# neka-nat/cupoch

Hardware: NVIDIA H100
Metric: icp_iterations_per_sec (higher is better)
Workload: dtype f32

## Files before the change

### cupoch_b200/csrc/icp.cu

```cuda
#include <float.h>
#include <math.h>
#include <stddef.h>
#include <stdlib.h>
#include <time.h>
#include <string.h>

#include "cphb_internal.cuh"
#include <vector>
#include "cphb_eigen3.cuh"

#include "icp_types.cuh"
#include "icp_solve.cuh"
#include "icp_rows.cuh"
#include "icp_kernels.cuh"
#include "icp_estimate.cuh"
#include "icp_aux.cuh"


struct cphb_icp {
    cphb_index *index;
    cphb_icp_params prm;
    cphb_cloud tgt;
    unsigned n_src, n_pad;
    unsigned n_full;
    void *arena;
    size_t arena_bytes;
    float4 *pristine_xyz, *pristine_nrm, *pristine_cov;
    float4 *work_xyz, *work_nrm, *work_cov;
    float4 *src_col;
    float4 *tix_nrm, *tix_grad, *tix_cov;
    float4 *alt_xyz, *alt_nrm, *alt_cov, *alt_col, *cur_col;
    int2 *alt_prev;
    uint32_t *rt_keys, *rt_keys2, *rt_vals, *rt_order;
    IcpState *st;
    IcpState *h_st;
    bool owns_host;
    cudaEvent_t ev0, ev1;
    double *partials;
    int32_t *corr_index;
    unsigned *cmp_counts;
    unsigned *cmp_total;
    double *tile_sums;
    unsigned *flag_bits;
    unsigned flag_words;
    int2 *prev;
    unsigned *dbg = nullptr;
    cudaEvent_t *dbg_ev = nullptr;
    unsigned grid_search;
    unsigned grid;
    unsigned reduce_grid;
    cudaStream_t stream;
};

struct HostCache {
    IcpState *h_st = nullptr;
    cudaEvent_t ev0 = nullptr, ev1 = nullptr;
    bool in_use = false;
};
static thread_local HostCache t_cache;
static thread_local cudaEvent_t t_source_ready = nullptr;
struct SideStream {
    cudaStream_t stream = nullptr;
    cudaEvent_t fork = nullptr, join = nullptr;
    int device = -1;
};
static thread_local SideStream t_side;

static bool is_identity4(const float *T) {
// ... 193 lines not shown
    }
    const bool want_nrm = params->estimation == CPHB_EST_SYMMETRIC && source->normals;
    const bool want_col = params->estimation == CPHB_EST_COLORED_ICP && source->colors;
    const bool want_cov = params->estimation == CPHB_EST_GENERALIZED_ICP && source->covariances;
    size_t off = 0;
    auto take = [&](size_t bytes) { size_t o = off; off = cphb_align(off + bytes, 256); return o; };
    size_t o_pxyz = take(sizeof(float4) * n_pad), o_wxyz = take(sizeof(float4) * n_pad);
    size_t o_pnrm = want_nrm ? take(sizeof(float4) * n_pad) : 0, o_wnrm = want_nrm ? take(sizeof(float4) * n_pad) : 0;
    size_t o_pcov = want_cov ? take(sizeof(float4) * 3 * n_pad) : 0, o_wcov = want_cov ? take(sizeof(float4) * 3 * n_pad) : 0;
    size_t o_col = want_col ? take(sizeof(float4) * n_pad) : 0;
    size_t o_st = take(sizeof(IcpState));
    size_t o_part = take(sizeof(double) * 32 * (icp->reduce_grid > icp->grid ? icp->reduce_grid : icp->grid));
    const size_t nt_pad = (size_t)icp->index->v.n_leaves * CPHB_LEAF;
    const int est = params->estimation;
    const bool t_nrm = target->normals && (est == CPHB_EST_POINT_TO_PLANE || est == CPHB_EST_SYMMETRIC || est == CPHB_EST_COLORED_ICP);
    const bool t_grad = target->color_gradient && est == CPHB_EST_COLORED_ICP;
    const bool t_cov = target->covariances && est == CPHB_EST_GENERALIZED_ICP;
    size_t o_tn = t_nrm ? take(sizeof(float4) * (nt_pad ? nt_pad : 1)) : 0, o_tg = t_grad ? take(sizeof(float4) * (nt_pad ? nt_pad : 1)) : 0;
    size_t o_tc = t_cov ? take(sizeof(float4) * 3 * (nt_pad ? nt_pad : 1)) : 0;
    size_t o_ts = take(sizeof(double) * n_pad);
    const unsigned flag_words = n_pad / 1024 + 1;
    size_t o_fb = take(sizeof(unsigned) * 2 * flag_words);
    size_t o_prev = take(sizeof(int2) * n_pad);
    size_t o_axyz = take(sizeof(float4) * n_pad), o_aprev = take(sizeof(int2) * n_pad);
    size_t o_anrm = want_nrm ? take(sizeof(float4) * n_pad) : 0, o_acov = want_cov ? take(sizeof(float4) * 3 * n_pad) : 0;
    size_t o_acol = want_col ? take(sizeof(float4) * n_pad) : 0, o_ccol = want_col ? take(sizeof(float4) * n_pad) : 0;
    size_t o_rt = take(sizeof(uint32_t) * 4 * n_pad);
    const unsigned nf_pad = (unsigned)cphb_align(n_full ? n_full : 1, ICP_BLOCK);
    size_t o_ci = take(sizeof(int32_t) * nf_pad);
    unsigned cmp_blocks = (nf_pad + CMP_BLOCK - 1) / CMP_BLOCK;
    size_t o_cc = take(sizeof(unsigned) * (cmp_blocks + 1));
    size_t o_ct = take(16);
    icp->arena_bytes = off;
    rc = cphb_alloc_async(&icp->arena, off, s);
    if (rc) { cphb_index_destroy(icp->index); delete icp; return rc; }
    char *b = (char *)icp->arena;
    icp->pristine_xyz = (float4 *)(b + o_pxyz);
    icp->work_xyz = (float4 *)(b + o_wxyz);
    icp->pristine_nrm = want_nrm ? (float4 *)(b + o_pnrm) : nullptr;
    icp->work_nrm = want_nrm ? (float4 *)(b + o_wnrm) : nullptr;
    icp->pristine_cov = want_cov ? (float4 *)(b + o_pcov) : nullptr;
    icp->work_cov = want_cov ? (float4 *)(b + o_wcov) : nullptr;
    icp->src_col = want_col ? (float4 *)(b + o_col) : nullptr;
    icp->st = (IcpState *)(b + o_st);
    icp->partials = (double *)(b + o_part);
    icp->tix_nrm = t_nrm ? (float4 *)(b + o_tn) : nullptr;
    icp->tix_grad = t_grad ? (float4 *)(b + o_tg) : nullptr;
    icp->tix_cov = t_cov ? (float4 *)(b + o_tc) : nullptr;
    icp->tile_sums = (double *)(b + o_ts);
    icp->flag_bits = (unsigned *)(b + o_fb);
    icp->flag_words = flag_words;
    icp->prev = (int2 *)(b + o_prev);
    icp->alt_xyz = (float4 *)(b + o_axyz);
    icp->alt_prev = (int2 *)(b + o_aprev);
    icp->alt_nrm = want_nrm ? (float4 *)(b + o_anrm) : nullptr;
    icp->alt_cov = want_cov ? (float4 *)(b + o_acov) : nullptr;
    icp->alt_col = want_col ? (float4 *)(b + o_acol) : nullptr;
    icp->cur_col = want_col ? (float4 *)(b + o_ccol) : nullptr;
    icp->rt_keys = (uint32_t *)(b + o_rt);
    icp->rt_keys2 = icp->rt_keys + n_pad;
    icp->rt_vals = icp->rt_keys + 2 * (size_t)n_pad;
    icp->rt_order = icp->rt_keys + 3 * (size_t)n_pad;
    icp->corr_index = (int32_t *)(b + o_ci);
    icp->cmp_counts = (unsigned *)(b + o_cc);
    icp->cmp_total = (unsigned *)(b + o_ct);
    if (!t_cache.in_use) {
        if (!t_cache.h_st) {
            CREATE_TRY(cudaMallocHost((void **)&t_cache.h_st, sizeof(IcpState)));
            CREATE_TRY(cudaEventCreate(&t_cache.ev0));
            CREATE_TRY(cudaEventCreate(&t_cache.ev1));
        }
        t_cache.in_use = true;
        icp->owns_host = false;
        icp->h_st = t_cache.h_st;
        icp->ev0 = t_cache.ev0;
// ... 39 lines not shown
    delete icp;
}

static void fill_args(const cphb_icp *icp, IcpArgs &a) {
    memset(&a, 0, sizeof(a));
    a.ix = icp->index->v;
    a.src = icp->work_xyz;
    a.src_nrm = icp->work_nrm;
    a.src_cov = icp->work_cov;
    a.src_col = icp->src_col;
    a.tgt_nrm = icp->tix_nrm;
    a.tgt_grad = icp->tix_grad;
    a.tgt_cov = icp->tix_cov;
    a.has_tgt_col = icp->tgt.colors != nullptr;
    a.st = icp->st;
    a.partials = icp->partials;
    a.tile_sums = icp->tile_sums;
    a.flag_bits = icp->flag_bits;
    a.flag_words = icp->flag_words;
    a.reduce_grid = icp->reduce_grid;
    a.helper_blocks = icp->grid >= 64 ? (icp->grid / 8 > 2 ? icp->grid / 8 : 2) : 0;
    if (const char *e = getenv("CPHB_HELPER_BLOCKS")) { int v = atoi(e); if (v >= 0 && (unsigned)v < icp->grid / 2) a.helper_blocks = (unsigned)v; }
    a.prev = icp->prev;
    a.n_src = icp->n_src;
    a.n_pad = icp->n_pad;
    a.n_total = icp->n_src;
    float r = icp->prm.max_correspondence_distance;
    a.r2 = (r > 0.f) ? r * r : 0.f;
    a.rel_fitness = icp->prm.relative_fitness;
    a.rel_rmse = icp->prm.relative_rmse;
    a.det_thresh = icp->prm.det_thresh;
    a.max_iter = icp->prm.max_iteration > 0 ? icp->prm.max_iteration : 0;
    float lg = icp->prm.lambda_geometric;
    if (lg < 0.f || lg > 1.0f) lg = 0.968f;
    a.sg = (float)sqrt((double)lg);
    float lp = (float)(1.0 - (double)lg);
    a.sp = (float)sqrt((double)lp);
    a.cert_gain = 4.f;
    a.cert_cap = 0.5f;
    if (const char *e = getenv("CPHB_CERT_GAIN")) a.cert_gain = (float)atof(e);
    if (const char *e = getenv("CPHB_CERT_CAP")) a.cert_cap = (float)atof(e);
    a.cert_cap_r = 0.25f * (r > 0.f ? r : 0.f);
    a.r_up = (float)(sqrt((double)a.r2) * 1.00002);
    a.dbg = icp->dbg;
    a.claim_max = 8u;
    if (const char *e = getenv("CPHB_CLAIM_MAX")) { int v = atoi(e); if (v >= 1 && v <= 1024) a.claim_max = (unsigned)v; }
// ... 22 lines not shown
    unsigned nb = (n + CMP_BLOCK - 1) / CMP_BLOCK;
    if (nb == 0) nb = 1;
    CPHB_LAUNCH(compact_count_kernel, nb, CMP_BLOCK, 0, s, icp->corr_index, n, icp->cmp_counts);
    CPHB_LAUNCH(compact_scan_kernel, 1, 1024, 0, s, icp->cmp_counts, nb, icp->cmp_total);
    CPHB_LAUNCH(compact_write_kernel, nb, CMP_BLOCK, 0, s, icp->corr_index, n, icp->cmp_counts, corr_out);
    CPHB_CHECK_LAUNCH();
    return CPHB_OK;
}

static int retile(cphb_icp *icp, IcpArgs &a, cudaStream_t s) {
    const unsigned n_pad = icp->n_pad, grid = n_pad / 256;
    const uint32_t n_tgt_pad = (uint32_t)icp->index->v.n_leaves * CPHB_LEAF;
    CPHB_LAUNCH(retile_key_kernel, grid, 256, 0, s, a.prev, icp->n_src, n_pad, n_tgt_pad, icp->rt_keys, icp->rt_vals);
    CPHB_CHECK_LAUNCH();
    int bits = 1;
    while (bits < 32 && ((uint64_t)1 << bits) < (uint64_t)(n_tgt_pad >> 5) + 2u) ++bits;
    int rc = cphb_sort_pairs_u32(icp->rt_keys, icp->rt_keys2, icp->rt_vals, icp->rt_order, n_pad, bits, s);
    if (rc) return rc;
    float4 *o_xyz = (a.src == icp->work_xyz) ? icp->alt_xyz : icp->work_xyz;
    int2 *o_prev = (a.prev == icp->prev) ? icp->alt_prev : icp->prev;
    float4 *o_nrm = a.src_nrm ? ((a.src_nrm == icp->work_nrm) ? icp->alt_nrm : icp->work_nrm) : nullptr;
    float4 *o_cov = a.src_cov ? ((a.src_cov == icp->work_cov) ? icp->alt_cov : icp->work_cov) : nullptr;
    float4 *o_col = a.src_col ? ((a.src_col == icp->alt_col) ? icp->cur_col : icp->alt_col) : nullptr;
    CPHB_LAUNCH(retile_gather_kernel, grid, 256, 0, s, icp->rt_order, n_pad, a.src, a.prev, a.src_nrm, a.src_col, a.src_cov,
                o_xyz, o_prev, o_nrm, o_col, o_cov);
    CPHB_CHECK_LAUNCH();
    a.src = o_xyz;
    a.prev = o_prev;
    a.src_nrm = o_nrm;
    a.src_cov = o_cov;
    a.src_col = o_col;
    return CPHB_OK;
}

extern "C" int cphb_icp_run(cphb_icp *icp, const float h_init[16], cphb_comm *comm, cphb_icp_result *h_result,
                            int32_t *corr_out, void *stream) {
    cudaStream_t s = (cudaStream_t)stream;
    if (!icp || !h_init || !h_result) {
        cphb_set_error("cphb_icp_run: null argument");
        return CPHB_ERR_INVALID;
    }
    int rc = reset_working_copy(icp, s);
    if (rc) return rc;
    IcpState *h = icp->h_st;
    memset(h, 0, sizeof(*h));
    memcpy(h->T, h_init, 64);
    memcpy(h->U, h_init, 64);
    h->apply_u = is_identity4(h_init) ? 0 : 1;
    CPHB_CUDA(cudaMemcpyAsync(icp->st, h, sizeof(IcpState), cudaMemcpyHostToDevice, s));
    static const bool dbg_cert = getenv("CPHB_DEBUG_CERT") != nullptr;
    if (dbg_cert) {
        if (!icp->dbg) CPHB_CUDA(cudaMalloc(&icp->dbg, sizeof(unsigned) * 256 + 128));
        CPHB_CUDA(cudaMemsetAsync(icp->dbg, 0, sizeof(unsigned) * 256 + 128, s));
        CPHB_CUDA(cudaMemsetAsync(icp->dbg + 256, 0xff, 8, s));
// ... 421 lines not shown
```

### cupoch_b200/csrc/icp_aux.cuh

```cuda
#pragma once

__global__ void __launch_bounds__(256) gather_source_kernel(const float *__restrict__ xyz, const float *__restrict__ nrm,
                                                            const float *__restrict__ col, const float *__restrict__ cov,
                                                            int cov_col_major, const uint32_t *__restrict__ perm_all,
                                                            unsigned lo, unsigned n, unsigned n_pad, float4 *o_xyz,
                                                            float4 *o_nrm, float4 *o_col, float4 *o_cov) {
    unsigned i = blockIdx.x * blockDim.x + threadIdx.x;
    if (i >= n_pad) return;
    const uint32_t *perm = perm_all + lo;
    if (i < n) {
        size_t j = perm[i];
        o_xyz[i] = make_float4(xyz[3 * j], xyz[3 * j + 1], xyz[3 * j + 2], __uint_as_float((unsigned)j));
        if (o_nrm) o_nrm[i] = make_float4(nrm[3 * j], nrm[3 * j + 1], nrm[3 * j + 2], 0.f);
        if (o_col) o_col[i] = make_float4(col[3 * j], col[3 * j + 1], col[3 * j + 2], 0.f);
        if (o_cov) {
            const float *c = cov + 9 * j;
            for (int r = 0; r < 3; ++r)
                o_cov[(size_t)r * n_pad + i] = cov_col_major ? make_float4(c[r], c[3 + r], c[6 + r], 0.f)
                                                             : make_float4(c[3 * r], c[3 * r + 1], c[3 * r + 2], 0.f);
        }
    } else {
        size_t j = n ? perm[n - 1] : 0;
        float4 p = n ? make_float4(xyz[3 * j], xyz[3 * j + 1], xyz[3 * j + 2], 0.f) : make_float4(0.f, 0.f, 0.f, 0.f);
        p.w = __uint_as_float(0xffffffffu);
// ... 28 lines not shown
#pragma unroll
        for (int r = 0; r < 3; ++r)
            o_cov[3 * p + r] = !real ? make_float4(0.f, 0.f, 0.f, 0.f)
                                     : cov_col_major ? make_float4(c[r], c[3 + r], c[6 + r], 0.f)
                                                     : make_float4(c[3 * r], c[3 * r + 1], c[3 * r + 2], 0.f);
    }
}

__global__ void __launch_bounds__(256) retile_key_kernel(const int2 *__restrict__ prev, unsigned n_src, unsigned n_pad,
                                                         uint32_t n_tgt_pad, uint32_t *keys, uint32_t *vals) {
    unsigned i = blockIdx.x * blockDim.x + threadIdx.x;
    if (i >= n_pad) return;
    uint32_t k = (n_tgt_pad >> 5) + 1u;
    if (i < n_src) {
        const int pp = prev[i].x;
        k = (pp >= 0) ? ((uint32_t)pp >> 5) : (n_tgt_pad >> 5);
    }
    keys[i] = k;
    vals[i] = i;
}
__global__ void __launch_bounds__(256) retile_gather_kernel(const uint32_t *__restrict__ order, unsigned n_pad,
                                                            const float4 *__restrict__ xyz, const int2 *__restrict__ prev,
                                                            const float4 *__restrict__ nrm, const float4 *__restrict__ col,
                                                            const float4 *__restrict__ cov, float4 *o_xyz, int2 *o_prev,
                                                            float4 *o_nrm, float4 *o_col, float4 *o_cov) {
    unsigned i = blockIdx.x * blockDim.x + threadIdx.x;
    if (i >= n_pad) return;
    const unsigned s = order[i];
    o_xyz[i] = xyz[s];
    o_prev[i] = prev[s];
    if (nrm) o_nrm[i] = nrm[s];
    if (col) o_col[i] = col[s];
    if (cov)
#pragma unroll
        for (int r = 0; r < 3; ++r) o_cov[(size_t)r * n_pad + i] = cov[(size_t)r * n_pad + s];
}

#define CMP_BLOCK 1024
__global__ void __launch_bounds__(CMP_BLOCK) compact_count_kernel(const int32_t *__restrict__ ci, unsigned n,
                                                                  unsigned *block_counts) {
    __shared__ unsigned s_w[32];
    unsigned i = blockIdx.x * CMP_BLOCK + threadIdx.x;
    bool v = i < n && ci[i] >= 0;
    unsigned m = __ballot_sync(CPHB_FULL, v);
    if (lane_id() == 0) s_w[threadIdx.x >> 5] = __popc(m);
    __syncthreads();
    if (threadIdx.x < 32) {
        unsigned c = s_w[threadIdx.x];
#pragma unroll
        for (int o = 16; o > 0; o >>= 1) c += __shfl_xor_sync(CPHB_FULL, c, o);
        if (threadIdx.x == 0) block_counts[blockIdx.x] = c;
    }
}
// ... 98 lines not shown
```

### cupoch_b200/csrc/icp_kernels.cuh

```cuda
#pragma once

__device__ __forceinline__ void prefetch_l1(const void *p) { asm volatile("prefetch.global.L1 [%0];" ::"l"(p)); }
__device__ __forceinline__ void cp_async_16(void *smem, const void *gmem) {
    asm volatile("cp.async.cg.shared.global [%0], [%1], 16;" ::"r"(smem_u32(smem)), "l"(gmem) : "memory");
}
__device__ __forceinline__ void cp_async_8(void *smem, const void *gmem) {
    asm volatile("cp.async.ca.shared.global [%0], [%1], 8;" ::"r"(smem_u32(smem)), "l"(gmem) : "memory");
}
__device__ __forceinline__ void cp_async_commit() { asm volatile("cp.async.commit_group;" ::: "memory"); }
__device__ __forceinline__ void cp_async_wait_0() { asm volatile("cp.async.wait_group 0;" ::: "memory"); }
template <int N>
__device__ __forceinline__ void cp_async_wait() { asm volatile("cp.async.wait_group %0;" ::"n"(N) : "memory"); }
#ifndef ICP_GD
#define ICP_GD 2
#endif
#define ICP_NS (2 * ICP_GD)
#ifndef ICP_DMMA
#define ICP_DMMA 1
#endif
#ifndef ICP_F2D_INT
#define ICP_F2D_INT 0
#endif
__device__ __forceinline__ double f2d(float f) {
#if ICP_F2D_INT
    const unsigned u = __float_as_uint(f);
    const unsigned a = u & 0x7fffffffu;
    if (a - 0x00800000u >= 0x7f000000u) {
        if (a == 0u) return __hiloint2double((int)u, 0);
        return (double)f;
    }
    return __hiloint2double((int)((u & 0x80000000u) | ((a >> 3) + 0x38000000u)), (int)(u << 29));
#else
    return (double)f;
#endif
}
__device__ __forceinline__ void dmma_8x8x4(double &c0, double &c1, double a, double b) {
    asm volatile("mma.sync.aligned.m8n8k4.row.col.f64.f64.f64.f64 {%0,%1}, {%2}, {%3}, {%0,%1};" : "+d"(c0), "+d"(c1) : "d"(a), "d"(b));
}
template <int KIND>
// ... 20 lines not shown
#endif
__device__ __forceinline__ void grid_dependency_wait() {
#if CPHB_PDL
    asm volatile("griddepcontrol.wait;" ::: "memory");
#endif
}
__device__ __forceinline__ void grid_dependency_trigger() {
#if CPHB_PDL
    asm volatile("griddepcontrol.launch_dependents;" ::: "memory");
#endif
}

__host__ __device__ constexpr int pair_jtj_a(int p) {
    return p < 6 ? 0 : p < 11 ? 1 : p < 15 ? 2 : p < 18 ? 3 : p < 20 ? 4 : p < 21 ? 5 : p < 27 ? p - 21 : p == 27 ? 6 : p == 28 ? 7 : 8;
}
__host__ __device__ constexpr int pair_jtj_b(int p) {
    return p < 6 ? p : p < 11 ? p - 5 : p < 15 ? p - 9 : p < 18 ? p - 12 : p < 20 ? p - 14 : p < 21 ? 5 : p < 28 ? 6 : 8;
}
__host__ __device__ constexpr int pair_p2p_a(int p) { return p < 6 ? p : p < 15 ? (p - 6) / 3 : p == 28 ? 7 : 8; }
__host__ __device__ constexpr int pair_p2p_b(int p) { return p < 6 ? 8 : p < 15 ? 3 + (p - 6) % 3 : 8; }
__host__ __device__ constexpr bool pair_live(bool p2p, int p) { return p2p ? (p < 15 || p == 28 || p == 29) : p < 30; }

template <int KIND>
__device__ __forceinline__ void load_tgt_ix(const IcpArgs &a, unsigned p, const float4 &tp, TgtVals &t) {
    t.vt[0] = tp.x; t.vt[1] = tp.y; t.vt[2] = tp.z;
    t.ok = true;
    if (KIND == CPHB_EST_POINT_TO_PLANE) t.ok = a.tgt_nrm != nullptr;
    if (KIND == CPHB_EST_SYMMETRIC) t.ok = a.tgt_nrm && a.src_nrm;
    if (KIND == CPHB_EST_COLORED_ICP) t.ok = a.tgt_nrm && a.has_tgt_col && a.src_col && a.tgt_grad;
    if (KIND == CPHB_EST_GENERALIZED_ICP) t.ok = a.tgt_cov && a.src_cov;
    if (!t.ok) return;
    if (KIND == CPHB_EST_POINT_TO_PLANE || KIND == CPHB_EST_SYMMETRIC || KIND == CPHB_EST_COLORED_ICP) {
        const float4 n4 = a.tgt_nrm[p];
        t.nt[0] = n4.x; t.nt[1] = n4.y; t.nt[2] = n4.z;
        t.it = n4.w;
    }
    if (KIND == CPHB_EST_COLORED_ICP) {
        const float4 g4 = a.tgt_grad[p];
        t.gt[0] = g4.x; t.gt[1] = g4.y; t.gt[2] = g4.z;
    }
    if (KIND == CPHB_EST_GENERALIZED_ICP) {
#pragma unroll
        for (int r = 0; r < 3; ++r) {
            const float4 c4 = a.tgt_cov[3 * (size_t)p + r];
            t.ct[3 * r] = c4.x; t.ct[3 * r + 1] = c4.y; t.ct[3 * r + 2] = c4.z;
        }
    }
}

struct LaunchCtx {
    float U[12];
    unsigned long long init;
    bool apply, materialize, write_corr, use_cert;
// ... 87 lines not shown
            const float area = fmaxf(ex * ey, fmaxf(ex * ez, ey * ez));
            if (margin > a.cert_cap * sqrtf(area * (1.f / 32.f))) margin = 0.f;
        }
    } else if (c.use_cert) {
        cert = slk > a.r_up;
        if (margin > a.cert_cap_r) margin = 0.f;
    }
    if (cert) margin = 0.f;
}

__device__ __forceinline__ void lane_store_match(const IcpArgs &a, const LaunchCtx &c, unsigned i, unsigned orig, bool in_range,
                                                 bool found, int pos, unsigned j, bool cert, float slk, unsigned best_hi,
                                                 unsigned m1, unsigned m2, unsigned rb) {
    if (a.prev && !a.step_mode) {
        const unsigned other = (found && m1 == best_hi) ? m2 : m1;
        const float l2 = __uint_as_float(min(other, rb));
        const float fresh = __fmul_rd(sqrt_approx(l2), 0.99999f);
        a.prev[i] = make_int2(found ? pos : -1, __float_as_int(cert ? slk : fresh));
    }
    if (c.write_corr && in_range) a.corr_index[orig] = found ? (int32_t)j : -1;
}

template <int KIND>
__device__ __forceinline__ void load_tgt_smem(const IcpArgs &a, const float4 *gat, int lane, const float4 &tp, TgtVals &t) {
    t.vt[0] = tp.x; t.vt[1] = tp.y; t.vt[2] = tp.z;
    t.ok = true;
    if (KIND == CPHB_EST_POINT_TO_PLANE) t.ok = a.tgt_nrm != nullptr;
    if (KIND == CPHB_EST_SYMMETRIC) t.ok = a.tgt_nrm && a.src_nrm;
    if (KIND == CPHB_EST_COLORED_ICP) t.ok = a.tgt_nrm && a.has_tgt_col && a.src_col && a.tgt_grad;
    if (KIND == CPHB_EST_GENERALIZED_ICP) t.ok = a.tgt_cov && a.src_cov;
    if (!t.ok) return;
    if (KIND == CPHB_EST_POINT_TO_PLANE || KIND == CPHB_EST_SYMMETRIC || KIND == CPHB_EST_COLORED_ICP) {
        const float4 n4 = gat[32 + lane];
        t.nt[0] = n4.x; t.nt[1] = n4.y; t.nt[2] = n4.z;
        t.it = n4.w;
    }
    if (KIND == CPHB_EST_COLORED_ICP) {
        const float4 g4 = gat[64 + lane];
        t.gt[0] = g4.x; t.gt[1] = g4.y; t.gt[2] = g4.z;
    }
    if (KIND == CPHB_EST_GENERALIZED_ICP) {
#pragma unroll
        for (int r = 0; r < 3; ++r) {
            const float4 c4 = gat[32 * (1 + r) + lane];
            t.ct[3 * r] = c4.x; t.ct[3 * r + 1] = c4.y; t.ct[3 * r + 2] = c4.z;
        }
    }
}
template <int KIND>
__device__ __forceinline__ void gather_issue(const IcpArgs &a, float4 *gat, int lane, int p) {
    if (p < 0) return;
    cp_async_16(&gat[lane], &a.ix.pts[p]);
    if ((KIND == CPHB_EST_POINT_TO_PLANE || KIND == CPHB_EST_SYMMETRIC || KIND == CPHB_EST_COLORED_ICP) && a.tgt_nrm)
        cp_async_16(&gat[32 + lane], &a.tgt_nrm[p]);
    if (KIND == CPHB_EST_COLORED_ICP && a.tgt_grad) cp_async_16(&gat[64 + lane], &a.tgt_grad[p]);
    if (KIND == CPHB_EST_GENERALIZED_ICP && a.tgt_cov)
#pragma unroll
        for (int r = 0; r < 3; ++r) cp_async_16(&gat[32 * (1 + r) + lane], &a.tgt_cov[3 * (size_t)p + r]);
}

template <int KIND, int NROWS>
__device__ __forceinline__ void lane_rows_vals(const IcpArgs &a, bool found, const TgtVals &t, const float4 &s,
                                               const float (&sn)[3], const float (&Cs)[9], unsigned i, float (&J)[NROWS][6],
                                               float (&r)[NROWS]) {
#pragma unroll
    for (int q = 0; q < NROWS; ++q) {
        r[q] = 0.f;
#pragma unroll
        for (int c = 0; c < 6; ++c) J[q][c] = 0.f;
    }
    if (found) {
        const float4 cs4 = (KIND == CPHB_EST_COLORED_ICP && a.src_col) ? a.src_col[i] : make_float4(0.f, 0.f, 0.f, 0.f);
        build_rows_vals<KIND, NROWS>(a.sg, a.sp, s.x, s.y, s.z, sn, cs4, Cs, t, J, r);
        drop_nonfinite_rows<NROWS>(J, r);
    }
}
template <int KIND, int NROWS>
__device__ __forceinline__ void lane_rows(const IcpArgs &a, bool found, unsigned pos, const float4 &tp, const float4 &s,
                                          const float (&sn)[3], const float (&Cs)[9], unsigned i, float (&J)[NROWS][6],
                                          float (&r)[NROWS]) {
#pragma unroll
    for (int q = 0; q < NROWS; ++q) {
        r[q] = 0.f;
#pragma unroll
        for (int c = 0; c < 6; ++c) J[q][c] = 0.f;
    }
    if (found) {
        TgtVals t;
        load_tgt_ix<KIND>(a, pos, tp, t);
        const float4 cs4 = (KIND == CPHB_EST_COLORED_ICP && a.src_col) ? a.src_col[i] : make_float4(0.f, 0.f, 0.f, 0.f);
        build_rows_vals<KIND, NROWS>(a.sg, a.sp, s.x, s.y, s.z, sn, cs4, Cs, t, J, r);
        drop_nonfinite_rows<NROWS>(J, r);
    }
}

template <int KIND, int TOP>
__device__ __forceinline__ bool search_tile(const IcpArgs &a, const LaunchCtx &c, WarpSearchC &w, double *rows, unsigned tile,
                                            float4 s, const int2 pv, double &acc) {
    constexpr int NROWS = (KIND == CPHB_EST_COLORED_ICP) ? 2 : (KIND == CPHB_EST_GENERALIZED_ICP) ? 3 : 1;
    constexpr bool P2P = (KIND == CPHB_EST_POINT_TO_POINT);
    const int lane = lane_id();
    const unsigned i = tile * 32 + lane;
    const unsigned orig = __float_as_uint(s.w);
    const bool in_range = i < a.n_src;
    const float ox = s.x, oy = s.y, oz = s.z;
    float sn[3] = {0.f, 0.f, 0.f};
    float Cs[9] = {0.f, 0.f, 0.f, 0.f, 0.f, 0.f, 0.f, 0.f, 0.f};
    lane_transform<KIND>(a, c, i, s, sn, Cs);
    lane_writeback<KIND>(a, c, i, s, sn, Cs);

    float4 tp = make_float4(0.f, 0.f, 0.f, 0.f);
    bool cert;
    float slk;
    lane_warm_start(a, c, in_range, s, ox, oy, oz, pv, tp, w.best, cert, slk, w.margin);
    const unsigned long long before = w.best;
    w.qx = s.x; w.qy = s.y; w.qz = s.z;
    w.m1 = 0x7f800000u;
    w.m2 = 0x7f800000u;
    w.valid = in_range && !cert;
    w.track = __any_sync(CPHB_FULL, w.valid && w.margin > 0.f);
    w.refresh();
    warp_update_bound(w);
    w.warm = __all_sync(CPHB_FULL, !w.valid || w.best < c.init);
    int pos = pv.x;
    const bool searched = __any_sync(CPHB_FULL, w.valid);
    if (searched) {
        warp_query_box(w);
        warp_nn_search<TOP>(a.ix, w);
        if (w.best != before) {
            pos = (int)a.ix.inv[(unsigned)(w.best & 0xffffffffull)];
            tp = a.ix.pts[pos];
        }
    }
    if (a.dbg) {
        const unsigned nc = __popc(__ballot_sync(CPHB_FULL, cert));
        if (lane == 0) {
            atomicAdd(&a.dbg[min(a.launch_idx, 63)], nc);
            if (!searched) atomicAdd(&a.dbg[64 + min(a.launch_idx, 63)], 1u);
        }
    }
    const bool found = in_range && (w.best != c.init);
    const unsigned j = (unsigned)(w.best & 0xffffffffull);
    const float d2 = __uint_as_float((unsigned)(w.best >> 32));
    lane_store_match(a, c, i, orig, in_range, found, pos, j, cert, slk, (unsigned)(w.best >> 32), w.m1, w.m2, w.rb);
    acc = 0.0;
    if (c.materialize) return !searched;

    float J[NROWS][6], r[NROWS];
    lane_rows<KIND, NROWS>(a, found, (unsigned)pos, tp, s, sn, Cs, i, J, r);
    const unsigned char(*pair)[2] = P2P ? c_pair_p2p : c_pair_jtj;
    const int ca = pair[lane][0], cb = pair[lane][1];
    const unsigned live = P2P ? c_live_p2p : c_live_jtj;
#pragma unroll
    for (int q = 0; q < NROWS; ++q) {
        double *my = rows + lane * ROW_STRIDE;
#pragma unroll
        for (int k = 0; k < 6; ++k) my[k] = f2d(J[q][k]);
        my[6] = f2d(r[q]);
        my[7] = (q == 0 && found) ? f2d(d2) : 0.0;
        my[8] = (q == 0 && found) ? 1.0 : 0.0;
        __syncwarp();
#pragma unroll 8
        for (int t = 0; t < 32; ++t) acc = fma(rows[t * ROW_STRIDE + ca], rows[t * ROW_STRIDE + cb], acc);
        __syncwarp();
    }
    if (!((live >> lane) & 1u)) acc = 0.0;
    return !searched;
}

template <int KIND>
__device__ void icp_static_tail(const IcpArgs &a, IcpState *st, double (*s_rowbuf)[32], SolveSmem &s_solve, unsigned *s_flag,
                                const double row, bool materialize, unsigned n_skipped_block);

template <int KIND, int BLOCK>
__device__ void icp_reduce_body(const IcpArgs &a, double (*s_acc)[32], unsigned *s_last, SolveSmem &s_solve);

template <int KIND, int TOP, int ROLE>
__global__ void __launch_bounds__(ICP_SEARCH_WARPS * 32, ROLE == 0 ? ICP_MIN_BLOCKS_SEARCH : ICP_MIN_BLOCKS)
icp_iteration_kernel(const __grid_constant__ IcpArgs a) {
    __shared__ __align__(16) float4 s_tile[ICP_SEARCH_WARPS][2 * CPHB_LEAF];
    __shared__ uint64_t s_bar[ICP_SEARCH_WARPS][2];
    __shared__ double s_rows[ICP_SEARCH_WARPS][32 * ROW_STRIDE];
    __shared__ SolveSmem s_solve;
    __shared__ unsigned s_flag;
    __shared__ __align__(16) unsigned char s_pipe[ICP_SEARCH_WARPS][ICP_NS * 32 * 24];
    constexpr int NG = (KIND == CPHB_EST_POINT_TO_POINT) ? 1 : (KIND == CPHB_EST_GENERALIZED_ICP) ? 4 : (KIND == CPHB_EST_COLORED_ICP) ? 3 : 2;
    __shared__ __align__(16) float4 s_gat[ICP_SEARCH_WARPS][ICP_GD * NG * 32];

    IcpState *st = a.st;
    const int warp = threadIdx.x >> 5, lane = lane_id();
    grid_dependency_wait();
    __shared__ unsigned s_hdr[16];
    if (threadIdx.x < 16) {
        const unsigned k = threadIdx.x;
        const unsigned *src = (k < 12) ? reinterpret_cast<const unsigned *>(&st->U[k])
                              : (k == 12) ? reinterpret_cast<const unsigned *>(&st->done)
                              : (k == 13) ? reinterpret_cast<const unsigned *>(&st->apply_u)
                              : (k == 14) ? reinterpret_cast<const unsigned *>(&st->static_sched)
                                          : reinterpret_cast<const unsigned *>(&st->flag_parity);
        s_hdr[k] = *(volatile const unsigned *)src;
    }
    __syncthreads();
    const int done = (int)s_hdr[12];
    const int apply_u = (int)s_hdr[13];
    const int static_word = (int)s_hdr[14];
    const unsigned flag_parity = s_hdr[15] & 1u;
    if (done == 2) return;
    LaunchCtx c;
    c.materialize = (done == 1);
    c.apply = a.step_mode ? true : (!c.materialize && apply_u != 0);
// ... 53 lines not shown
                    const bool skipped = search_tile<KIND, TOP>(a, c, w, s_rows[warp], t, s, pv, acc);
                    hrow += acc;
                    if (skipped) ++n_skip;
                    else if (lane == 0) atomicOr(&flag_next[wd], 1u << (t & 31));
                }
            }
            if (lane == 0) { dbg_time(a, 1, false); dbg_time(a, 10, false); }
            icp_static_tail<KIND>(a, st, (double(*)[32])s_pipe, s_solve, &s_flag, hrow, c.materialize, n_skip);
            return;
        }
#if ICP_DMMA
        double gc0 = 0.0, gc1 = 0.0;
        double d2acc = 0.0;
        float *stage = reinterpret_cast<float *>(s_rows[warp]);
#else
        double lacc[32];
#pragma unroll
        for (int p = 0; p < 32; ++p) lacc[p] = 0.0;
#endif
        double wrow = 0.0;
        unsigned n_skipped = 0;
        bool searched_inline = false;
        unsigned tile = gw;
        float4 *pipe_s = reinterpret_cast<float4 *>(s_pipe[warp]);
        int2 *pipe_pv = reinterpret_cast<int2 *>(s_pipe[warp] + ICP_NS * 32 * 16);
        auto stage_load = [&](unsigned t, int slot) {
            if (t < n_tiles) {
                cp_async_16(&pipe_s[slot * 32 + lane], &a.src[t * 32 + lane]);
                cp_async_8(&pipe_pv[slot * 32 + lane], &a.prev[t * 32 + lane]);
            }
        };
#pragma unroll
        for (int j = 0; j < ICP_NS; ++j) {
            stage_load(tile + (unsigned)j * main_warps, j);
            cp_async_commit();
        }
        cp_async_wait<ICP_NS - ICP_GD>();
#pragma unroll
        for (int j = 0; j < ICP_GD; ++j) {
            if (tile + (unsigned)j * main_warps < n_tiles) gather_issue<KIND>(a, s_gat[warp] + j * NG * 32, lane, pipe_pv[j * 32 + lane].x);
            cp_async_commit();
        }
        unsigned fw = (tile < n_tiles) ? __ldg(&flag_cur[tile >> 5]) : 0u;
        int slot = 0, gslot = 0;
        float4 cold_s = make_float4(0.f, 0.f, 0.f, 0.f);
        int2 cold_pv = make_int2(-1, 0);
        for (;;) {
        bool cold = false;
        for (; tile < n_tiles; tile += main_warps) {
            cp_async_wait<ICP_GD - 1>();
            const unsigned t1 = tile + main_warps, tg = tile + ICP_GD * main_warps, tn = tile + ICP_NS * main_warps;
            float4 *gat = s_gat[warp] + gslot * NG * 32;
            const float4 s0 = pipe_s[slot * 32 + lane];
            float4 s = s0;
            const int2 pv = pipe_pv[slot * 32 + lane];
            const bool flagged = (fw >> (tile & 31)) & 1u;
            if (t1 < n_tiles) fw = __ldg(&flag_cur[t1 >> 5]);
            float4 tp = gat[lane];
            TgtVals tv;
            load_tgt_smem<KIND>(a, gat, lane, tp, tv);
            stage_load(tn, slot);
            if (tg < n_tiles) gather_issue<KIND>(a, gat, lane, pipe_pv[((slot + ICP_GD) % ICP_NS) * 32 + lane].x);
            cp_async_commit();
            slot = (slot + 1) % ICP_NS;
            gslot = (gslot + 1) % ICP_GD;
            const unsigned i = tile * 32 + lane;
            const unsigned orig = __float_as_uint(s.w);
            const bool in_range = i < a.n_src;
            const float ox = s.x, oy = s.y, oz = s.z;
            float sn[3] = {0.f, 0.f, 0.f};
            float Cs[9] = {0.f, 0.f, 0.f, 0.f, 0.f, 0.f, 0.f, 0.f, 0.f};
            lane_transform<KIND>(a, c, i, s, sn, Cs);
            unsigned long long best;
            bool cert;
            float slk, margin;
            lane_warm_start<true>(a, c, in_range, s, ox, oy, oz, pv, tp, best, cert, slk, margin);
            if (flagged) continue;
            const bool need_search = __any_sync(CPHB_FULL, in_range && !cert);
            if (need_search) {
                cold = true;
                cold_s = s0;
                cold_pv = pv;
                break;
            }
            ++n_skipped;
            lane_writeback<KIND>(a, c, i, s, sn, Cs);
            if (a.dbg) {
                const unsigned nc = __popc(__ballot_sync(CPHB_FULL, cert));
                if (lane == 0) {
                    atomicAdd(&a.dbg[min(a.launch_idx, 63)], nc);
                    atomicAdd(&a.dbg[64 + min(a.launch_idx, 63)], 1u);
                }
            }
            const bool found = in_range && (best != c.init);
            const unsigned j = (unsigned)(best & 0xffffffffull);
            const float d2 = __uint_as_float((unsigned)(best >> 32));
            lane_store_match(a, c, i, orig, in_range, found, pv.x, j, true, slk, (unsigned)(best >> 32), 0x7f800000u,
                             0x7f800000u, (unsigned)(best >> 32));
            if (c.materialize) continue;
            float J[NROWS][6], r[NROWS];
            lane_rows_vals<KIND, NROWS>(a, found, tv, s, sn, Cs, i, J, r);
#if ICP_DMMA
#pragma unroll
            for (int q = 0; q < NROWS; ++q) {
                __syncwarp();
                *reinterpret_cast<float4 *>(stage + lane * 8) = make_float4(J[q][0], J[q][1], J[q][2], J[q][3]);
                *reinterpret_cast<float4 *>(stage + lane * 8 + 4) = make_float4(J[q][4], J[q][5], r[q], (q == 0 && found) ? 1.f : 0.f);
                __syncwarp();
#pragma unroll
                for (int m4 = 0; m4 < 8; ++m4) {
                    const double x = f2d(stage[(4 * m4 + (lane & 3)) * 8 + (lane >> 2)]);
                    dmma_8x8x4(gc0, gc1, x, x);
                }
            }
            if (found) d2acc += f2d(d2);
#else
#pragma unroll
            for (int q = 0; q < NROWS; ++q) {
// ... 306 lines not shown
```

### cupoch_b200/csrc/icp_types.cuh

```cuda
#pragma once

#define ICP_BLOCK 256
#define ICP_WARPS (ICP_BLOCK / 32)
#define ROW_STRIDE 9

struct IcpState {
    double total[32];
    double local[32];
    float T[16];
    float U[16];
    float fitness, rmse;
    int done;
    int iterations;
    int converged;
    int apply_u;
    unsigned ticket;
    unsigned tile_counter;
    unsigned cert_tiles;
    int static_sched;
    int tail_done;
    unsigned block_ticket;
    unsigned flag_parity;
    long long n_corr;
    unsigned comm_timeout;
    unsigned pad_local;
    unsigned pad_;
};

struct IcpArgs {
    IndexView ix;
    float4 *src;
    float4 *src_nrm;
    float4 *src_cov;
    const float4 *src_col;
    const float4 *tgt_nrm, *tgt_grad, *tgt_cov;
    int has_tgt_col;
    IcpState *st;
    double *partials;
    double *tile_sums;
    unsigned *flag_bits;
    unsigned flag_words;
    unsigned helper_blocks;
    unsigned reduce_grid;
    int2 *prev;
    float cert_gain;
    float cert_cap;
    float cert_cap_r;
    float r_up;
    unsigned *dbg;
    unsigned claim_max;
    int static_sched;
    int32_t *corr_index;
    unsigned long long n_total;
    unsigned n_src, n_pad;
    float r2;
    float rel_fitness, rel_rmse, det_thresh, sg, sp;
    int launch_idx, max_iter;
    int defer_finalize;
    int use_p2p;
    P2pView p2p;
    int step_mode;
    int tmax;
};

__constant__ unsigned char c_pair_jtj[32][2] = {
    {0, 0}, {0, 1}, {0, 2}, {0, 3}, {0, 4}, {0, 5}, {1, 1}, {1, 2}, {1, 3}, {1, 4}, {1, 5},
    {2, 2}, {2, 3}, {2, 4}, {2, 5}, {3, 3}, {3, 4}, {3, 5}, {4, 4}, {4, 5}, {5, 5},
    {0, 6}, {1, 6}, {2, 6}, {3, 6}, {4, 6}, {5, 6}, {6, 6}, {7, 8}, {8, 8}, {8, 8}, {8, 8}};
__constant__ unsigned char c_pair_p2p[32][2] = {
    {0, 8}, {1, 8}, {2, 8}, {3, 8}, {4, 8}, {5, 8}, {0, 3}, {0, 4}, {0, 5}, {1, 3}, {1, 4},
    {1, 5}, {2, 3}, {2, 4}, {2, 5}, {8, 8}, {8, 8}, {8, 8}, {8, 8}, {8, 8}, {8, 8},
    {8, 8}, {8, 8}, {8, 8}, {8, 8}, {8, 8}, {8, 8}, {8, 8}, {7, 8}, {8, 8}, {8, 8}, {8, 8}};
__constant__ unsigned c_live_jtj = 0x3fffffffu;
__constant__ unsigned c_live_p2p = 0x00007fffu | (1u << 28) | (1u << 29);

#ifdef __CUDACC__
__device__ __forceinline__ unsigned long long gtime() {
    unsigned long long t;
    asm volatile("mov.u64 %0, %globaltimer;" : "=l"(t));
    return t;
}
__device__ __forceinline__ void dbg_time(const IcpArgs &a, int slot, bool take_min) {
    if (!a.dbg || a.launch_idx != 20) return;
    unsigned long long *p = reinterpret_cast<unsigned long long *>(a.dbg + 256) + slot;
    if (take_min) atomicMin(p, gtime());
    else atomicMax(p, gtime());
// ... 3 lines not shown
```

Before: 7211.

## Cache matched target attributes per source point in a compact coalesced mrow buffer

Adds a per-source 'mrow' buffer that stores the matched target's position and attributes (normal, gradient, covariance) packed by source index. It is written only when the nearest neighbour changes and is permuted along with the other arrays during retiling. The main loop now streams these rows with coalesced cp.async as part of the source pipeline, replacing the dependent two-stage gather of target data through prev indices. The pipeline depth is set to 3 stages. This costs extra memory, extra scattered writes when a match moves, and larger retile traffic, and it fetches the correspondence index from the target point's w field.

```diff
diff --git a/cupoch_b200/csrc/icp.cu b/cupoch_b200/csrc/icp.cu
--- a/cupoch_b200/csrc/icp.cu
+++ b/cupoch_b200/csrc/icp.cu
@@ -31,6 +31,7 @@
     float4 *tix_nrm, *tix_grad, *tix_cov;
     float4 *alt_xyz, *alt_nrm, *alt_cov, *alt_col, *cur_col;
     int2 *alt_prev;
+    float4 *alt_mrow;
     uint32_t *rt_keys, *rt_keys2, *rt_vals, *rt_order;
     IcpState *st;
     IcpState *h_st;
@@ -44,6 +45,7 @@
     unsigned *flag_bits;
     unsigned flag_words;
     int2 *prev;
+    float4 *mrow;
     unsigned *dbg = nullptr;
     cudaEvent_t *dbg_ev = nullptr;
     unsigned grid_search;
@@ -283,6 +285,8 @@
     const unsigned flag_words = n_pad / 1024 + 1;
     size_t o_fb = take(sizeof(unsigned) * 2 * flag_words);
     size_t o_prev = take(sizeof(int2) * n_pad);
+    const size_t mrow_b = (size_t)mrow_bytes(est) * n_pad;
+    size_t o_mrow = take(mrow_b), o_amrow = take(mrow_b);
     size_t o_axyz = take(sizeof(float4) * n_pad), o_aprev = take(sizeof(int2) * n_pad);
     size_t o_anrm = want_nrm ? take(sizeof(float4) * n_pad) : 0, o_acov = want_cov ? take(sizeof(float4) * 3 * n_pad) : 0;
     size_t o_acol = want_col ? take(sizeof(float4) * n_pad) : 0, o_ccol = want_col ? take(sizeof(float4) * n_pad) : 0;
@@ -312,6 +316,8 @@
     icp->flag_bits = (unsigned *)(b + o_fb);
     icp->flag_words = flag_words;
     icp->prev = (int2 *)(b + o_prev);
+    icp->mrow = (float4 *)(b + o_mrow);
+    icp->alt_mrow = (float4 *)(b + o_amrow);
     icp->alt_xyz = (float4 *)(b + o_axyz);
     icp->alt_prev = (int2 *)(b + o_aprev);
     icp->alt_nrm = want_nrm ? (float4 *)(b + o_anrm) : nullptr;
@@ -397,6 +403,7 @@
     a.helper_blocks = icp->grid >= 64 ? (icp->grid / 8 > 2 ? icp->grid / 8 : 2) : 0;
     if (const char *e = getenv("CPHB_HELPER_BLOCKS")) { int v = atoi(e); if (v >= 0 && (unsigned)v < icp->grid / 2) a.helper_blocks = (unsigned)v; }
     a.prev = icp->prev;
+    a.mrow = icp->mrow;
     a.n_src = icp->n_src;
     a.n_pad = icp->n_pad;
     a.n_total = icp->n_src;
@@ -465,14 +472,17 @@
     float4 *o_nrm = a.src_nrm ? ((a.src_nrm == icp->work_nrm) ? icp->alt_nrm : icp->work_nrm) : nullptr;
     float4 *o_cov = a.src_cov ? ((a.src_cov == icp->work_cov) ? icp->alt_cov : icp->work_cov) : nullptr;
     float4 *o_col = a.src_col ? ((a.src_col == icp->alt_col) ? icp->cur_col : icp->alt_col) : nullptr;
+    float4 *o_mrow = (a.mrow == icp->mrow) ? icp->alt_mrow : icp->mrow;
+    const int est = icp->prm.estimation;
     CPHB_LAUNCH(retile_gather_kernel, grid, 256, 0, s, icp->rt_order, n_pad, a.src, a.prev, a.src_nrm, a.src_col, a.src_cov,
-                o_xyz, o_prev, o_nrm, o_col, o_cov);
+                a.mrow, mrow_q4(est), mrow_h2(est), o_xyz, o_prev, o_nrm, o_col, o_cov, o_mrow);
     CPHB_CHECK_LAUNCH();
     a.src = o_xyz;
     a.prev = o_prev;
     a.src_nrm = o_nrm;
     a.src_cov = o_cov;
     a.src_col = o_col;
+    a.mrow = o_mrow;
     return CPHB_OK;
 }
 
diff --git a/cupoch_b200/csrc/icp_aux.cuh b/cupoch_b200/csrc/icp_aux.cuh
--- a/cupoch_b200/csrc/icp_aux.cuh
+++ b/cupoch_b200/csrc/icp_aux.cuh
@@ -74,13 +74,17 @@
 __global__ void __launch_bounds__(256) retile_gather_kernel(const uint32_t *__restrict__ order, unsigned n_pad,
                                                             const float4 *__restrict__ xyz, const int2 *__restrict__ prev,
                                                             const float4 *__restrict__ nrm, const float4 *__restrict__ col,
-                                                            const float4 *__restrict__ cov, float4 *o_xyz, int2 *o_prev,
-                                                            float4 *o_nrm, float4 *o_col, float4 *o_cov) {
+                                                            const float4 *__restrict__ cov, const float4 *__restrict__ mrow,
+                                                            int mrow_q4, int mrow_h2, float4 *o_xyz, int2 *o_prev,
+                                                            float4 *o_nrm, float4 *o_col, float4 *o_cov, float4 *o_mrow) {
     unsigned i = blockIdx.x * blockDim.x + threadIdx.x;
     if (i >= n_pad) return;
     const unsigned s = order[i];
     o_xyz[i] = xyz[s];
     o_prev[i] = prev[s];
+    for (int q = 0; q < mrow_q4; ++q) o_mrow[(size_t)q * n_pad + i] = mrow[(size_t)q * n_pad + s];
+    if (mrow_h2)
+        reinterpret_cast<float2 *>(o_mrow + (size_t)mrow_q4 * n_pad)[i] = reinterpret_cast<const float2 *>(mrow + (size_t)mrow_q4 * n_pad)[s];
     if (nrm) o_nrm[i] = nrm[s];
     if (col) o_col[i] = col[s];
     if (cov)
diff --git a/cupoch_b200/csrc/icp_kernels.cuh b/cupoch_b200/csrc/icp_kernels.cuh
--- a/cupoch_b200/csrc/icp_kernels.cuh
+++ b/cupoch_b200/csrc/icp_kernels.cuh
@@ -11,10 +11,9 @@
 __device__ __forceinline__ void cp_async_wait_0() { asm volatile("cp.async.wait_group 0;" ::: "memory"); }
 template <int N>
 __device__ __forceinline__ void cp_async_wait() { asm volatile("cp.async.wait_group %0;" ::"n"(N) : "memory"); }
-#ifndef ICP_GD
-#define ICP_GD 2
-#endif
-#define ICP_NS (2 * ICP_GD)
+#ifndef ICP_NS
+#define ICP_NS 3
+#endif
 #ifndef ICP_DMMA
 #define ICP_DMMA 1
 #endif
@@ -81,13 +80,17 @@
 __host__ __device__ constexpr bool pair_live(bool p2p, int p) { return p2p ? (p < 15 || p == 28 || p == 29) : p < 30; }
 
 template <int KIND>
+__device__ __forceinline__ bool tgt_ok(const IcpArgs &a) {
+    if (KIND == CPHB_EST_POINT_TO_PLANE) return a.tgt_nrm != nullptr;
+    if (KIND == CPHB_EST_SYMMETRIC) return a.tgt_nrm && a.src_nrm;
+    if (KIND == CPHB_EST_COLORED_ICP) return a.tgt_nrm && a.has_tgt_col && a.src_col && a.tgt_grad;
+    if (KIND == CPHB_EST_GENERALIZED_ICP) return a.tgt_cov && a.src_cov;
+    return true;
+}
+template <int KIND>
 __device__ __forceinline__ void load_tgt_ix(const IcpArgs &a, unsigned p, const float4 &tp, TgtVals &t) {
     t.vt[0] = tp.x; t.vt[1] = tp.y; t.vt[2] = tp.z;
-    t.ok = true;
-    if (KIND == CPHB_EST_POINT_TO_PLANE) t.ok = a.tgt_nrm != nullptr;
-    if (KIND == CPHB_EST_SYMMETRIC) t.ok = a.tgt_nrm && a.src_nrm;
-    if (KIND == CPHB_EST_COLORED_ICP) t.ok = a.tgt_nrm && a.has_tgt_col && a.src_col && a.tgt_grad;
-    if (KIND == CPHB_EST_GENERALIZED_ICP) t.ok = a.tgt_cov && a.src_cov;
+    t.ok = tgt_ok<KIND>(a);
     if (!t.ok) return;
     if (KIND == CPHB_EST_POINT_TO_PLANE || KIND == CPHB_EST_SYMMETRIC || KIND == CPHB_EST_COLORED_ICP) {
         const float4 n4 = a.tgt_nrm[p];
@@ -221,41 +224,52 @@
 }
 
 template <int KIND>
-__device__ __forceinline__ void load_tgt_smem(const IcpArgs &a, const float4 *gat, int lane, const float4 &tp, TgtVals &t) {
-    t.vt[0] = tp.x; t.vt[1] = tp.y; t.vt[2] = tp.z;
-    t.ok = true;
-    if (KIND == CPHB_EST_POINT_TO_PLANE) t.ok = a.tgt_nrm != nullptr;
-    if (KIND == CPHB_EST_SYMMETRIC) t.ok = a.tgt_nrm && a.src_nrm;
-    if (KIND == CPHB_EST_COLORED_ICP) t.ok = a.tgt_nrm && a.has_tgt_col && a.src_col && a.tgt_grad;
-    if (KIND == CPHB_EST_GENERALIZED_ICP) t.ok = a.tgt_cov && a.src_cov;
+__device__ __forceinline__ void mrow_store(const IcpArgs &a, unsigned i, const TgtVals &t) {
+    constexpr int Q4 = mrow_q4(KIND);
+    float4 q[Q4];
+    q[0] = make_float4(t.vt[0], t.vt[1], t.vt[2], 0.f);
+    float2 h = make_float2(0.f, 0.f);
+    if constexpr (KIND == CPHB_EST_POINT_TO_PLANE || KIND == CPHB_EST_SYMMETRIC) {
+        q[0].w = t.nt[0];
+        h = make_float2(t.nt[1], t.nt[2]);
+    }
+    if constexpr (KIND == CPHB_EST_COLORED_ICP) {
+        q[0].w = t.nt[0];
+        q[1] = make_float4(t.nt[1], t.nt[2], t.it, t.gt[0]);
+        h = make_float2(t.gt[1], t.gt[2]);
+    }
+    if constexpr (KIND == CPHB_EST_GENERALIZED_ICP) {
+        q[0].w = t.ct[0];
+        q[1] = make_float4(t.ct[1], t.ct[2], t.ct[3], t.ct[4]);
+        q[2] = make_float4(t.ct[5], t.ct[6], t.ct[7], t.ct[8]);
+    }
+#pragma unroll
+    for (int k = 0; k < Q4; ++k) a.mrow[(size_t)k * a.n_pad + i] = q[k];
+    if constexpr (mrow_h2(KIND) != 0) reinterpret_cast<float2 *>(a.mrow + (size_t)Q4 * a.n_pad)[i] = h;
+}
+template <int KIND>
+__device__ __forceinline__ void mrow_unpack(const IcpArgs &a, const float4 *q4, const float2 *h2, int lane, TgtVals &t) {
+    const float4 q0 = q4[lane];
+    t.vt[0] = q0.x; t.vt[1] = q0.y; t.vt[2] = q0.z;
+    t.ok = tgt_ok<KIND>(a);
     if (!t.ok) return;
-    if (KIND == CPHB_EST_POINT_TO_PLANE || KIND == CPHB_EST_SYMMETRIC || KIND == CPHB_EST_COLORED_ICP) {
-        const float4 n4 = gat[32 + lane];
-        t.nt[0] = n4.x; t.nt[1] = n4.y; t.nt[2] = n4.z;
-        t.it = n4.w;
-    }
-    if (KIND == CPHB_EST_COLORED_ICP) {
-        const float4 g4 = gat[64 + lane];
-        t.gt[0] = g4.x; t.gt[1] = g4.y; t.gt[2] = g4.z;
-    }
-    if (KIND == CPHB_EST_GENERALIZED_ICP) {
-#pragma unroll
-        for (int r = 0; r < 3; ++r) {
-            const float4 c4 = gat[32 * (1 + r) + lane];
-            t.ct[3 * r] = c4.x; t.ct[3 * r + 1] = c4.y; t.ct[3 * r + 2] = c4.z;
-        }
-    }
-}
-template <int KIND>
-__device__ __forceinline__ void gather_issue(const IcpArgs &a, float4 *gat, int lane, int p) {
-    if (p < 0) return;
-    cp_async_16(&gat[lane], &a.ix.pts[p]);
-    if ((KIND == CPHB_EST_POINT_TO_PLANE || KIND == CPHB_EST_SYMMETRIC || KIND == CPHB_EST_COLORED_ICP) && a.tgt_nrm)
-        cp_async_16(&gat[32 + lane], &a.tgt_nrm[p]);
-    if (KIND == CPHB_EST_COLORED_ICP && a.tgt_grad) cp_async_16(&gat[64 + lane], &a.tgt_grad[p]);
-    if (KIND == CPHB_EST_GENERALIZED_ICP && a.tgt_cov)
-#pragma unroll
-        for (int r = 0; r < 3; ++r) cp_async_16(&gat[32 * (1 + r) + lane], &a.tgt_cov[3 * (size_t)p + r]);
+    if constexpr (KIND == CPHB_EST_POINT_TO_PLANE || KIND == CPHB_EST_SYMMETRIC) {
+        const float2 h = h2[lane];
+        t.nt[0] = q0.w; t.nt[1] = h.x; t.nt[2] = h.y;
+    }
+    if constexpr (KIND == CPHB_EST_COLORED_ICP) {
+        const float4 q1 = q4[32 + lane];
+        const float2 h = h2[lane];
+        t.nt[0] = q0.w; t.nt[1] = q1.x; t.nt[2] = q1.y;
+        t.it = q1.z;
+        t.gt[0] = q1.w; t.gt[1] = h.x; t.gt[2] = h.y;
+    }
+    if constexpr (KIND == CPHB_EST_GENERALIZED_ICP) {
+        const float4 q1 = q4[32 + lane], q2 = q4[64 + lane];
+        t.ct[0] = q0.w;
+        t.ct[1] = q1.x; t.ct[2] = q1.y; t.ct[3] = q1.z; t.ct[4] = q1.w;
+        t.ct[5] = q2.x; t.ct[6] = q2.y; t.ct[7] = q2.z; t.ct[8] = q2.w;
+    }
 }
 
 template <int KIND, int NROWS>
@@ -269,24 +283,6 @@
         for (int c = 0; c < 6; ++c) J[q][c] = 0.f;
     }
     if (found) {
-        const float4 cs4 = (KIND == CPHB_EST_COLORED_ICP && a.src_col) ? a.src_col[i] : make_float4(0.f, 0.f, 0.f, 0.f);
-        build_rows_vals<KIND, NROWS>(a.sg, a.sp, s.x, s.y, s.z, sn, cs4, Cs, t, J, r);
-        drop_nonfinite_rows<NROWS>(J, r);
-    }
-}
-template <int KIND, int NROWS>
-__device__ __forceinline__ void lane_rows(const IcpArgs &a, bool found, unsigned pos, const float4 &tp, const float4 &s,
-                                          const float (&sn)[3], const float (&Cs)[9], unsigned i, float (&J)[NROWS][6],
-                                          float (&r)[NROWS]) {
-#pragma unroll
-    for (int q = 0; q < NROWS; ++q) {
-        r[q] = 0.f;
-#pragma unroll
-        for (int c = 0; c < 6; ++c) J[q][c] = 0.f;
-    }
-    if (found) {
-        TgtVals t;
-        load_tgt_ix<KIND>(a, pos, tp, t);
         const float4 cs4 = (KIND == CPHB_EST_COLORED_ICP && a.src_col) ? a.src_col[i] : make_float4(0.f, 0.f, 0.f, 0.f);
         build_rows_vals<KIND, NROWS>(a.sg, a.sp, s.x, s.y, s.z, sn, cs4, Cs, t, J, r);
         drop_nonfinite_rows<NROWS>(J, r);
@@ -322,6 +318,7 @@
     warp_update_bound(w);
     w.warm = __all_sync(CPHB_FULL, !w.valid || w.best < c.init);
     int pos = pv.x;
+    bool moved = false;
     const bool searched = __any_sync(CPHB_FULL, w.valid);
     if (searched) {
         warp_query_box(w);
@@ -329,6 +326,7 @@
         if (w.best != before) {
             pos = (int)a.ix.inv[(unsigned)(w.best & 0xffffffffull)];
             tp = a.ix.pts[pos];
+            moved = true;
         }
     }
     if (a.dbg) {
@@ -345,8 +343,11 @@
     acc = 0.0;
     if (c.materialize) return !searched;
 
+    TgtVals tv;
+    if (found) load_tgt_ix<KIND>(a, (unsigned)pos, tp, tv);
+    if (moved && found && a.mrow && !a.step_mode) mrow_store<KIND>(a, i, tv);
     float J[NROWS][6], r[NROWS];
-    lane_rows<KIND, NROWS>(a, found, (unsigned)pos, tp, s, sn, Cs, i, J, r);
+    lane_rows_vals<KIND, NROWS>(a, found, tv, s, sn, Cs, i, J, r);
     const unsigned char(*pair)[2] = P2P ? c_pair_p2p : c_pair_jtj;
     const int ca = pair[lane][0], cb = pair[lane][1];
     const unsigned live = P2P ? c_live_p2p : c_live_jtj;
@@ -382,9 +383,7 @@
     __shared__ double s_rows[ICP_SEARCH_WARPS][32 * ROW_STRIDE];
     __shared__ SolveSmem s_solve;
     __shared__ unsigned s_flag;
-    __shared__ __align__(16) unsigned char s_pipe[ICP_SEARCH_WARPS][ICP_NS * 32 * 24];
-    constexpr int NG = (KIND == CPHB_EST_POINT_TO_POINT) ? 1 : (KIND == CPHB_EST_GENERALIZED_ICP) ? 4 : (KIND == CPHB_EST_COLORED_ICP) ? 3 : 2;
-    __shared__ __align__(16) float4 s_gat[ICP_SEARCH_WARPS][ICP_GD * NG * 32];
+    __shared__ __align__(16) unsigned char s_pipe[ICP_SEARCH_WARPS][ICP_NS * 32 * (24 + mrow_bytes(KIND))];
 
     IcpState *st = a.st;
     const int warp = threadIdx.x >> 5, lane = lane_id();
@@ -484,12 +483,20 @@
         unsigned n_skipped = 0;
         bool searched_inline = false;
         unsigned tile = gw;
+        constexpr int Q4 = mrow_q4(KIND);
         float4 *pipe_s = reinterpret_cast<float4 *>(s_pipe[warp]);
-        int2 *pipe_pv = reinterpret_cast<int2 *>(s_pipe[warp] + ICP_NS * 32 * 16);
+        float4 *pipe_m4 = pipe_s + ICP_NS * 32;
+        int2 *pipe_pv = reinterpret_cast<int2 *>(pipe_m4 + ICP_NS * Q4 * 32);
+        float2 *pipe_m2 = reinterpret_cast<float2 *>(pipe_pv + ICP_NS * 32);
+        const float2 *mrow2 = reinterpret_cast<const float2 *>(a.mrow + (size_t)Q4 * a.n_pad);
         auto stage_load = [&](unsigned t, int slot) {
             if (t < n_tiles) {
-                cp_async_16(&pipe_s[slot * 32 + lane], &a.src[t * 32 + lane]);
-                cp_async_8(&pipe_pv[slot * 32 + lane], &a.prev[t * 32 + lane]);
+                const unsigned k = t * 32 + lane;
+                cp_async_16(&pipe_s[slot * 32 + lane], &a.src[k]);
+#pragma unroll
+                for (int q = 0; q < Q4; ++q) cp_async_16(&pipe_m4[(slot * Q4 + q) * 32 + lane], &a.mrow[(size_t)q * a.n_pad + k]);
+                cp_async_8(&pipe_pv[slot * 32 + lane], &a.prev[k]);
+                if constexpr (mrow_h2(KIND) != 0) cp_async_8(&pipe_m2[slot * 32 + lane], &mrow2[k]);
             }
         };
 #pragma unroll
@@ -497,35 +504,26 @@
             stage_load(tile + (unsigned)j * main_warps, j);
             cp_async_commit();
         }
-        cp_async_wait<ICP_NS - ICP_GD>();
-#pragma unroll
-        for (int j = 0; j < ICP_GD; ++j) {
-            if (tile + (unsigned)j * main_warps < n_tiles) gather_issue<KIND>(a, s_gat[warp] + j * NG * 32, lane, pipe_pv[j * 32 + lane].x);
-            cp_async_commit();
-        }
         unsigned fw = (tile < n_tiles) ? __ldg(&flag_cur[tile >> 5]) : 0u;
-        int slot = 0, gslot = 0;
+        int slot = 0;
         float4 cold_s = make_float4(0.f, 0.f, 0.f, 0.f);
         int2 cold_pv = make_int2(-1, 0);
         for (;;) {
         bool cold = false;
         for (; tile < n_tiles; tile += main_warps) {
-            cp_async_wait<ICP_GD - 1>();
-            const unsigned t1 = tile + main_warps, tg = tile + ICP_GD * main_warps, tn = tile + ICP_NS * main_warps;
-            float4 *gat = s_gat[warp] + gslot * NG * 32;
+            cp_async_wait<ICP_NS - 1>();
+            const unsigned t1 = tile + main_warps, tn = tile + ICP_NS * main_warps;
             const float4 s0 = pipe_s[slot * 32 + lane];
             float4 s = s0;
             const int2 pv = pipe_pv[slot * 32 + lane];
             const bool flagged = (fw >> (tile & 31)) & 1u;
             if (t1 < n_tiles) fw = __ldg(&flag_cur[t1 >> 5]);
-            float4 tp = gat[lane];
             TgtVals tv;
-            load_tgt_smem<KIND>(a, gat, lane, tp, tv);
+            mrow_unpack<KIND>(a, pipe_m4 + slot * Q4 * 32, pipe_m2 + slot * 32, lane, tv);
+            float4 tp = make_float4(tv.vt[0], tv.vt[1], tv.vt[2], 0.f);
             stage_load(tn, slot);
-            if (tg < n_tiles) gather_issue<KIND>(a, gat, lane, pipe_pv[((slot + ICP_GD) % ICP_NS) * 32 + lane].x);
             cp_async_commit();
             slot = (slot + 1) % ICP_NS;
-            gslot = (gslot + 1) % ICP_GD;
             const unsigned i = tile * 32 + lane;
             const unsigned orig = __float_as_uint(s.w);
             const bool in_range = i < a.n_src;
@@ -555,7 +553,7 @@
                 }
             }
             const bool found = in_range && (best != c.init);
-            const unsigned j = (unsigned)(best & 0xffffffffull);
+            const unsigned j = (found && c.write_corr) ? __float_as_uint(a.ix.pts[pv.x].w) : 0u;
             const float d2 = __uint_as_float((unsigned)(best >> 32));
             lane_store_match(a, c, i, orig, in_range, found, pv.x, j, true, slk, (unsigned)(best >> 32), 0x7f800000u,
                              0x7f800000u, (unsigned)(best >> 32));
diff --git a/cupoch_b200/csrc/icp_types.cuh b/cupoch_b200/csrc/icp_types.cuh
--- a/cupoch_b200/csrc/icp_types.cuh
+++ b/cupoch_b200/csrc/icp_types.cuh
@@ -43,6 +43,7 @@
     unsigned helper_blocks;
     unsigned reduce_grid;
     int2 *prev;
+    float4 *mrow;
     float cert_gain;
     float cert_cap;
     float cert_cap_r;
@@ -62,6 +63,14 @@
     int step_mode;
     int tmax;
 };
+
+__host__ __device__ constexpr int mrow_q4(int kind) {
+    return kind == CPHB_EST_COLORED_ICP ? 2 : kind == CPHB_EST_GENERALIZED_ICP ? 3 : 1;
+}
+__host__ __device__ constexpr int mrow_h2(int kind) {
+    return (kind == CPHB_EST_POINT_TO_PLANE || kind == CPHB_EST_SYMMETRIC || kind == CPHB_EST_COLORED_ICP) ? 1 : 0;
+}
+__host__ __device__ constexpr int mrow_bytes(int kind) { return 16 * mrow_q4(kind) + 8 * mrow_h2(kind); }
 
 __constant__ unsigned char c_pair_jtj[32][2] = {
     {0, 0}, {0, 1}, {0, 2}, {0, 3}, {0, 4}, {0, 5}, {1, 1}, {1, 2}, {1, 3}, {1, 4}, {1, 5},
```

Result: faster. 7546 (median of 6 runs) (+4.7%).
